# leavesnight/VIEO_SLAM

Hardware: AMD Instinct MI355X
Metric: frontend+localBA frames/sec on EuRoC MH05 stereo-VIO; ATE vs ref (higher is better)
Workload: dtype u8 (extract/match) + f64 (pose optimisation)

## Files before the change

### vieo_slam_amd/csrc/pose_opt_vio.hip

```cpp
#pragma clang fp contract(fast)

#include <type_traits>
#include <vector>

#include "imu_device.h"

namespace vieo {

constexpr double kCosH[9] = {1.0, -0.125, 0.0026041666666666665, -2.170138888888889e-05, 9.68812003968254e-08, -2.691144455467372e-10, 5.096864498991235e-13, -7.001187498614334e-16, 7.292903644389931e-19};
constexpr double kSinHT[9] = {0.5, -0.020833333333333332, 0.00026041666666666666, -1.5500992063492063e-06, 5.382288910934745e-09, -1.2232474797578965e-11, 1.9603324996120133e-14, -2.333729166204778e-17, 2.1449716601146855e-20};
constexpr double kJrA[9] = {0.5, -0.041666666666666664, 0.001388888888888889, -2.48015873015873e-05, 2.755731922398589e-07, -2.08767569878681e-09, 1.1470745597729725e-11, -4.779477332387385e-14, 1.5619206968586225e-16};
constexpr double kJrB[9] = {0.16666666666666666, -0.008333333333333333, 0.0001984126984126984, -2.7557319223985893e-06, 2.505210838544172e-08, -1.6059043836821613e-10, 7.647163731819816e-13, -2.8114572543455206e-15, 8.22063524662433e-18};
constexpr double kAtanQ[16] = {0.3333333333333333, -0.2, 0.14285714285714285, -0.1111111111111111, 0.09090909090909091, -0.07692307692307693, 0.06666666666666667, -0.058823529411764705, 0.05263157894736842, -0.047619047619047616, 0.043478260869565216, -0.04, 0.037037037037037035, -0.034482758620689655, 0.03225806451612903, -0.030303030303030304};
__device__ __forceinline__ Qd q_renorm(const Qd& q, bool& ok) {
  const double e = (q.w * q.w + q.x * q.x + q.y * q.y + q.z * q.z) - 1.0;
  ok = ok && fabs(e) < 1e-5;
  const double r = 1.0 - e * (0.5 - 0.375 * e);
  return Qd{q.w * r, q.x * r, q.y * r, q.z * r};
}
template <int N>
__device__ __forceinline__ double horner(const double (&c)[N], double u) {
  double r = c[N - 1];
#pragma unroll
  for (int k = N - 2; k >= 0; k--) r = __builtin_fma(r, u, c[k]);
  return r;
}
__device__ __forceinline__ double rcp_nr(double d) {
  double inv = __builtin_amdgcn_rcp(d);
  inv = __builtin_fma(__builtin_fma(-d, inv, 1.0), inv, inv);
  return __builtin_fma(__builtin_fma(-d, inv, 1.0), inv, inv);
}
__device__ __forceinline__ Qd so3_exp_unit(const double* w, bool& ok) {
  const double u = w[0] * w[0] + w[1] * w[1] + w[2] * w[2];
  ok = ok && u < 0.25;
  const double real = horner(kCosH, u), imag = horner(kSinHT, u);
  return q_renorm(Qd{real, imag * w[0], imag * w[1], imag * w[2]}, ok);
}
__device__ __forceinline__ void so3_log_unit(const Qd& q, double* out, double* g, bool& ok) {
  const double n2 = q.x * q.x + q.y * q.y + q.z * q.z, w2 = q.w * q.w;
  ok = ok && n2 < 0.0625 * w2;
  const double iw = rcp_nr(q.w), x2 = n2 * (iw * iw);
  const double Q = horner(kAtanQ, x2), P = __builtin_fma(-x2, Q, 1.0);
  const double f = 2.0 * P * iw;
  out[0] = f * q.x, out[1] = f * q.y, out[2] = f * q.z;
  *g = Q * rcp_nr(4.0 * P * P);
}
__device__ __noinline__ double so3_JrInv_g_of(const double* e) {
  const double th2 = e[0] * e[0] + e[1] * e[1] + e[2] * e[2], th = sqrt(th2);
  if (th < 1e-5) return 1. / 12.;
  double sth, cth;
  sincos(th, &sth, &cth);
  return (1.0 - (1.0 + cth) * th / (2.0 * sth)) / th2;
}
__device__ __forceinline__ void so3_JrInv_g(const double* e, double g, double* J) {
  const double xx = e[0] * e[0], yy = e[1] * e[1], zz = e[2] * e[2];
  const double xy = g * e[0] * e[1], xz = g * e[0] * e[2], yz = g * e[1] * e[2];
  J[0] = 1.0 - g * (yy + zz), J[1] = xy - 0.5 * e[2], J[2] = xz + 0.5 * e[1];
  J[3] = xy + 0.5 * e[2], J[4] = 1.0 - g * (xx + zz), J[5] = yz - 0.5 * e[0];
  J[6] = xz - 0.5 * e[1], J[7] = yz + 0.5 * e[0], J[8] = 1.0 - g * (xx + yy);
}
__device__ __forceinline__ void so3_Jr_unit(const double* w, double* J) {
  const double u = w[0] * w[0] + w[1] * w[1] + w[2] * w[2];
  const double A = horner(kJrA, u), B = horner(kJrB, u);
  const double xx = w[0] * w[0], yy = w[1] * w[1], zz = w[2] * w[2];
  const double xy = B * w[0] * w[1], xz = B * w[0] * w[2], yz = B * w[1] * w[2];
  J[0] = 1.0 - B * (yy + zz), J[1] = xy + A * w[2], J[2] = xz - A * w[1];
  J[3] = xy - A * w[2], J[4] = 1.0 - B * (xx + zz), J[5] = yz + A * w[0];
  J[6] = xz + A * w[1], J[7] = yz - A * w[0], J[8] = 1.0 - B * (xx + yy);
}
struct RotCache {
  Qd qe, qb;
  double g_e;
  double w[3];
  Qd qp;
  double g_p;
  int w_small;
};

__device__ __forceinline__ void prior_error(const NSd& pr, const NSd& si, double* err, RotCache& C) {
  double Rb[9], d[3];
  q_to_R(q_of(pr), Rb);
  for (int k = 0; k < 3; k++) d[k] = si.p[k] - pr.p[k];
  mTv3(Rb, d, err);
  bool ok = true;
  Qd q = q_renorm(q_mul(q_conj(q_of(pr)), q_of(si)), ok);
  double g;
  so3_log_unit(q, err + 6, &g, ok);
  for (int k = 0; k < 3; k++) {
    err[3 + k] = si.v[k] - pr.v[k];
    err[9 + k] = si.bg[k] + si.dbg[k] - (pr.bg[k] + pr.dbg[k]);
    err[12 + k] = si.ba[k] + si.dba[k] - (pr.ba[k] + pr.dba[k]);
  }
  if (!ok) {
    q = q_norm(q_mul(q_conj(q_of(pr)), q_of(si)));
    so3_log_q(q, err + 6);
    g = so3_JrInv_g_of(err + 6);
  }
  C.qp = q, C.g_p = g;
}
__device__ __forceinline__ void prior_jacobian_init(double* J, int tid, int nthreads) {
  for (int e = tid; e < 225; e += nthreads) {
    const int r = e / 15, c = e - r * 15;
    J[e] = (r == c && ((r >= 3 && r < 6) || r >= 9)) ? 1.0 : 0.0;
  }
}
__device__ __forceinline__ void prior_linearize(const double* err, double* J, const RotCache& C) {
  double tmp[9], Jrinv[9];
  q_to_R(C.qp, tmp);
  set3(J, 15, 0, 0, tmp, 1.0);
  so3_JrInv_g(err + 6, C.g_p, Jrinv);
  set3(J, 15, 6, 6, Jrinv, 1.0);
}

__device__ __forceinline__ void imu_error_rot(const vieo_imu_preint& M, const Qd& qRij, const NSd& si, const NSd& sj, double* err, RotCache& C) {
  double w[3];
  mv3(M.JgR, si.dbg, w);
  bool ok = true;
  const Qd qx = so3_exp_unit(w, ok);
  const bool w_small = ok;
  Qd qb = q_renorm(q_mul(q_conj(q_of(si)), q_of(sj)), ok);
  const Qd qa = q_renorm(q_mul(qRij, qx), ok);
  Qd qe = q_renorm(q_mul(q_conj(qa), qb), ok);
  double g;
  so3_log_unit(qe, err + 6, &g, ok);
  if (!ok) {
    qb = q_norm(q_mul(q_conj(q_of(si)), q_of(sj)));
    qe = q_norm(q_mul(q_conj(q_norm(q_mul(qRij, so3_exp_q(w)))), qb));
    so3_log_q(qe, err + 6);
    g = so3_JrInv_g_of(err + 6);
  }
  C.qe = qe, C.qb = qb, C.g_e = g;
  C.w[0] = w[0], C.w[1] = w[1], C.w[2] = w[2], C.w_small = w_small ? 1 : 0;
}
__device__ __forceinline__ void imu_jacobian_init(const vieo_imu_preint& M, double* J, int tid, int nthreads) {
  for (int e = tid; e < 9 * 24; e += nthreads) {
    const int r = e / 24, c = e - r * 24;
    double v = 0.0;
    if (r < 3) {
      if (c >= 9 && c < 12) v = (c - 9 == r) ? -1.0 : 0.0;
      if (c >= 18 && c < 21) v = -M.Jgp[r * 3 + c - 18];
      if (c >= 21) v = -M.Jap[r * 3 + c - 21];
    } else if (r < 6) {
      if (c >= 18 && c < 21) v = -M.Jgv[(r - 3) * 3 + c - 18];
      if (c >= 21) v = -M.Jav[(r - 3) * 3 + c - 21];
    }
    J[e] = v;
  }
}
__device__ __forceinline__ void imu_linearize_pv(const vieo_imu_preint& M, const double* gw, const NSd& si, const NSd& sj, double* J) {
  const int ld = 24, cj = 0, ci = 9, idR = 6, idV = 3;
  double Ri[9], RiT[9], Rj[9], t[3], r[3], Hm[9], tmp[9];
  q_to_R(q_of(si), Ri);
// ... 242 lines not shown
struct VioShared {
  NSd nsj, nsi, bkj, bki, prior;
  union {
    struct {
      double H[900], L[900];
    };
    struct {
      double cov[225], C[225], E[225], Cinv[225 * 2];
    };
  };
  double b[32], x[32], tr_tail[64];
  double red[4 * 28], vis[28];
  double errI[9], errB[6], errP[15], wI[9], wP[15];
  double JI[9 * 24], JP[225], InfoI[81], T[225], TP[225], Hp[225];
  double chiq[8];
  double xv[4];
  int xfail;
  RotCache rc;
  double qRij[4];
  double gw[4];
  vieo_imu_preint imu;
  int ok;
};

struct VioEncShared {
  double Info[36], err[6], we[6], chi, J[6 * 12], T[6 * 12];
};

__device__ __noinline__ void vio_enc_setup(const vieo_pose_enc* pe, VioEncShared* S) {
  double M[6][12];
  for (int i = 0; i < 6; i++)
    for (int j = 0; j < 6; j++) M[i][j] = pe->enc.Sigma[i * 6 + j], M[i][6 + j] = (i == j) ? 1.0 : 0.0;
  for (int c = 0; c < 6; c++) {
    int piv = c;
    for (int r = c + 1; r < 6; r++)
      if (fabs(M[r][c]) > fabs(M[piv][c])) piv = r;
    if (piv != c)
      for (int j = 0; j < 12; j++) {
        const double t = M[c][j];
        M[c][j] = M[piv][j], M[piv][j] = t;
      }
    const double d = M[c][c];
    for (int j = 0; j < 12; j++) M[c][j] /= d;
    for (int r = 0; r < 6; r++)
      if (r != c) {
        const double f = M[r][c];
// ... 46 lines not shown
  asm volatile(
      "global_load_dwordx4 %0, %16, off sc0 sc1\n\t"
      "global_load_dwordx4 %1, %16, off offset:512 sc0 sc1\n\t"
      "global_load_dwordx4 %2, %16, off offset:1024 sc0 sc1\n\t"
      "global_load_dwordx4 %3, %16, off offset:1536 sc0 sc1\n\t"
      "global_load_dwordx4 %4, %16, off offset:2048 sc0 sc1\n\t"
      "global_load_dwordx4 %5, %16, off offset:2560 sc0 sc1\n\t"
      "global_load_dwordx4 %6, %16, off offset:3072 sc0 sc1\n\t"
      "global_load_dwordx4 %7, %16, off offset:3584 sc0 sc1\n\t"
      "global_load_dwordx4 %8, %17, off sc0 sc1\n\t"
      "global_load_dwordx4 %9, %17, off offset:512 sc0 sc1\n\t"
      "global_load_dwordx4 %10, %17, off offset:1024 sc0 sc1\n\t"
      "global_load_dwordx4 %11, %17, off offset:1536 sc0 sc1\n\t"
      "global_load_dwordx4 %12, %17, off offset:2048 sc0 sc1\n\t"
      "global_load_dwordx4 %13, %17, off offset:2560 sc0 sc1\n\t"
      "global_load_dwordx4 %14, %17, off offset:3072 sc0 sc1\n\t"
      "global_load_dwordx4 %15, %17, off offset:3584 sc0 sc1\n\t"
      "s_waitcnt vmcnt(0)"
      : "=&v"(v[0]), "=&v"(v[1]), "=&v"(v[2]), "=&v"(v[3]), "=&v"(v[4]), "=&v"(v[5]), "=&v"(v[6]), "=&v"(v[7]), "=&v"(v[8]), "=&v"(v[9]), "=&v"(v[10]), "=&v"(v[11]), "=&v"(v[12]), "=&v"(v[13]), "=&v"(v[14]), "=&v"(v[15])
      : "v"(p), "v"(p2)
      : "memory");
}
template <int BS, bool MC, bool ENC>
__global__ void __launch_bounds__(BS)
k_pose_opt_vio(const vieo_vio_frame* __restrict__ frames, const vieo_pose_obs* __restrict__ obs_all,
               uint8_t* __restrict__ outlier_all, vieo_vio_result* __restrict__ results, int other_launched,
               PoseXchg* __restrict__ xchg, unsigned launch_id) {
  __shared__ VioShared S;
  __shared__ double s_tr[BS == 64 ? 1 : 28 * (BS / 32) * 34];
  __shared__ double s_xf[MC ? 48 * (BS / 64) : 1];
  __shared__ __align__(8) unsigned char s_cam_store[sizeof(CamD) * (MC ? 4 : 1)];
  CamD* s_cams = reinterpret_cast<CamD*>(s_cam_store);
  __shared__ __align__(8) unsigned char s_enc_store[ENC ? sizeof(VioEncShared) : 8];
  VioEncShared* SE = reinterpret_cast<VioEncShared*>(s_enc_store);
  __shared__ __align__(16) vieo_pose_obs s_obs[(BS == 256 && !MC) ? 768 : 1];
  __shared__ uint8_t s_lvl[(BS == 256 && !MC) ? 768 : 4];
  const int f = blockIdx.x, tid = threadIdx.x, lane = tid & 63, wave = tid >> 6;
  const int T1 = BS > 64 ? 64 : 0, T2 = BS > 128 ? 128 : 0;
  const int T3 = BS > 192 ? 192 : 0;
  const vieo_vio_frame& F = frames[f];
  const int N = F.base.n_obs;
  constexpr int kVioSplitObs = 768;
  constexpr int kVioReplicaMinObs = 700;
  const vieo_pose_obs* obs = obs_all + F.base.obs_begin;
  uint8_t* outl = outlier_all + F.base.obs_begin;
  vieo_vio_result* R = results + f;
  const vieo_pose_enc* pe = F.base.enc;
  const bool cam_other = (F.base.n_cams > 0) != MC, enc_other = (pe != nullptr && pe->enc.dt != 0) != ENC;
  if ((cam_other && (other_launched & 1)) || (enc_other && (other_launched & 2))) return;
  const bool other_kind = cam_other || enc_other;
  bool bad_cams = other_kind;
  if (MC && !other_kind) {
    if (tid == 0) S.ok = !(F.base.n_cams > 4 || !F.base.cams);
    __syncthreads();
    if (tid < 4 && S.ok)
      if (!cam_from_abi(F.base.cams[tid < F.base.n_cams ? tid : 0], s_cams[tid])) S.ok = 0;
    __syncthreads();
    bad_cams = !S.ok;
    __syncthreads();
  }
  if (bad_cams || (N < 3 && !F.no_mps) || N > kVioMaxObs) {
    for (int i = tid; i < N; i += BS) outl[i] = 0;
    for (int i = tid; i < 225; i += BS) R->H_marg[i] = 0;
    if (tid == 0) {
      R->base.nav = F.base.nav;
      R->base.n_inliers = 0;
      R->base.status = bad_cams ? VIEO_E_INVALID : N > kVioMaxObs ? VIEO_E_CAPACITY : VIEO_POSE_TOO_FEW;
      R->base.lm_iterations = 0;
      R->base.reserved = 0;
      R->has_marg = 0;
      R->reserved = 0;
    }
    return;
  }
  CamD c;
  c.fx = F.base.fx, c.fy = F.base.fy, c.cx = F.base.cx, c.cy = F.base.cy, c.bf = F.base.bf;
  for (int i = 0; i < 9; i++) c.Rcb[i] = F.base.Rcb[i];
  for (int i = 0; i < 3; i++) c.tcb[i] = F.base.tcb[i];
  const bool fixedLast = !F.last_has_prior, hasImu = F.imu.dt != 0;
  const int n = fixedLast ? 15 : 30;
  const bool bodom = hasImu || ENC;
  if (tid == 0) {
    ns_load(S.nsj, F.base.nav);
    ns_load(S.nsi, F.nav_last);
    ns_load(S.prior, F.nav_prior);
  }
  if (ENC && tid == T2) vio_enc_setup(pe, SE);
  if (hasImu && wave == 0) {
    double* M = S.Cinv;
    for (int e = lane; e < 9 * 18; e += 64) {
      const int i = e / 18, j = e % 18;
      M[e] = j < 9 ? F.imu.Sigma[i * 9 + j] : (j - 9 == i ? 1.0 : 0.0);
    }
    wave_sync();
    for (int cidx = 0; cidx < 9; cidx++) {
      int piv = cidx;
      double best = fabs(M[cidx * 18 + cidx]);
      for (int r = cidx + 1; r < 9; r++)
        if (fabs(M[r * 18 + cidx]) > best) best = fabs(M[r * 18 + cidx]), piv = r;
      if (piv != cidx) {
        if (lane < 18) {
// ... 4 lines not shown
        wave_sync();
      }
      const double d = M[cidx * 18 + cidx];
      wave_sync();
      if (lane < 18) M[cidx * 18 + lane] /= d;
      wave_sync();
      double fr[3];
      for (int h = 0; h < 3; h++) {
        const int e = lane + 64 * h;
        fr[h] = e < 162 ? M[(e / 18) * 18 + cidx] : 0;
      }
      wave_sync();
      for (int h = 0; h < 3; h++) {
        const int e = lane + 64 * h;
        if (e < 162 && e / 18 != cidx) M[e] -= fr[h] * M[cidx * 18 + e % 18];
      }
      wave_sync();
    }
    for (int e = lane; e < 81; e += 64) S.InfoI[e] = M[(e / 9) * 18 + 9 + e % 9] * (fixedLast ? 1e-2 : 1.0);
  }
  if (!fixedLast)
    for (int e = tid; e < 225; e += BS) S.Hp[e] = F.H_prior[e];
  if (tid < 3) S.gw[tid] = F.gw[tid];
  prior_jacobian_init(S.JP, tid, BS);
  if (hasImu) imu_jacobian_init(F.imu, S.JI, tid, BS);
  if (tid == BS - 1 && hasImu) {
    const Qd q = R_to_q(F.imu.Rij);
    S.qRij[0] = q.w, S.qRij[1] = q.x, S.qRij[2] = q.y, S.qRij[3] = q.z;
  }
  for (int e = tid; e < (int)(offsetof(vieo_imu_preint, Sigma) / 8); e += BS)
    reinterpret_cast<double*>(&S.imu)[e] = reinterpret_cast<const double*>(&F.imu)[e];
  __syncthreads();
  if (BS == 256) {
    for (int i = tid; i < 900; i += BS) S.H[i] = 0.0;
    __syncthreads();
  }
  const double deltatij = F.imu.dt ? F.imu.dt : F.dt_frames;
  const double infoBg = F.inv_sigma_bg2 / deltatij * (fixedLast ? 1e-2 : 1.0);
  const double infoBa = F.inv_sigma_ba2 / deltatij * (fixedLast ? 1e-2 : 1.0);
  const double dI = sqrt(16.919), dB = sqrt(12.592), dP = sqrt(25.0), dE = sqrt(12.592);
  const double deltaMono = (double)(float)sqrt(5.991), deltaStereo = (double)(float)sqrt(7.815);
  const float chi2Mono = 5.991f, chi2Stereo = 7.815f;
  auto optimise = [&](auto vt_c, auto g_c) __attribute__((always_inline)) {
  constexpr int VT = decltype(vt_c)::value;
  constexpr int G = decltype(g_c)::value;
  const int g = G > 1 ? (int)blockIdx.y : 0;
  const int Nv = tid < VT ? N : 0;
  const int i0 = g * VT + tid;
// ... 71 lines not shown
        v[tid] = t;
      }
    }
    epoch++;
    __syncthreads();
    if (S.xfail && tid < 64) {
      const unsigned long long pz = (unsigned long long)(((launch_id & 0xFFFFFu) << 12) | 0xFFFu) << 32;
      xq_t pq;
      pq.x = pz, pq.y = pz;
      xq_store(&xb->cell[tid >> 5][g][tid & 31], pq);
    }
  };
  unsigned long long levelmask = 0;
  bool vis_robust = true;
  int nBad = 0, total_iters = 0, total_trials = 0;
  const int n_edges_total = N + (hasImu ? 1 : 0) + 1 + (fixedLast ? 0 : 1) + (ENC ? 1 : 0);
  double rhoE = 1.0;

#ifdef VIEO_POSE_PROBE
  unsigned long long pp_last = __builtin_amdgcn_s_memtime();
#endif
  constexpr int VTE = kObsLds ? 128 : VT;
  auto all_errors = [&](double* rhoI, double* rhoB, double* rhoP, bool with_visual, double* vis) -> double {
    if (with_visual && tid < VTE) {
      Est e;
      e.p[0] = S.nsj.p[0], e.p[1] = S.nsj.p[1], e.p[2] = S.nsj.p[2];
      e.qw = S.nsj.qw, e.qx = S.nsj.qx, e.qy = S.nsj.qy, e.qz = S.nsj.qz;
      PoseXf X;
      make_xf(c, e, X);
      rig_xf(X, e.p);
      double tc = 0;
      if constexpr (kObsLds) {
        const int K = (N + VTE - 1) / VTE;
        auto slots = [&](int k0, auto u_c) __attribute__((always_inline)) {
          constexpr int U = decltype(u_c)::value;
          VisFlat E[U];
          bool valid[U];
#pragma unroll
          for (int u = 0; u < U; u++) {
            const int i = min(tid + (k0 + u) * VTE, N - 1);
            valid[u] = tid + (k0 + u) * VTE < N && !s_lvl[i];
            vis_error_flat(c, X, s_obs[i], valid[u], E[u]);
          }
#pragma unroll
          for (int u = 0; u < U; u++) {
            double r0, r1;
// ... 14 lines not shown
        double err[3], Pc[3];
        const double chi2 = edge_eval<MC>(c, s_cams, X, e.p, o, err, Pc, nullptr, MC ? s_xf + (VT == BS ? 0 : 48 * wave) : nullptr);
        double r0 = chi2, r1 = 1.;
        if (vis_robust) {
          const double dl = o.ur >= 0 ? deltaStereo : deltaMono;
          huber(chi2, dl, dl * dl, &r0, &r1);
        }
        tc += r0;
      }
      }
      tc = BS == 64 ? wave_sum_d_bfly(tc) : wave_sum_d(tc);
      if (lane == 0) S.red[wave] = tc;
    }
    if (BS > 192) {
      if (VT > 128) {
        if (tid == T3 && hasImu) {
          RT(17, imu_error(S.imu, S.gw, S.nsi, S.nsj, S.errI, 6, 1);
             imu_error_rot(S.imu, Qd{S.qRij[0], S.qRij[1], S.qRij[2], S.qRij[3]}, S.nsi, S.nsj, S.errI, S.rc));
        }
      } else {
        if (tid == T3 && hasImu) RT(17, imu_error_rot(S.imu, Qd{S.qRij[0], S.qRij[1], S.qRij[2], S.qRij[3]}, S.nsi, S.nsj, S.errI, S.rc));
        if (tid == T2 && hasImu) RT(18, imu_error(S.imu, S.gw, S.nsi, S.nsj, S.errI, 6, 1));
      }
    } else if (tid == 0 && hasImu) {
      imu_error(S.imu, S.gw, S.nsi, S.nsj, S.errI, 6, 1);
      imu_error_rot(S.imu, Qd{S.qRij[0], S.qRij[1], S.qRij[2], S.qRij[3]}, S.nsi, S.nsj, S.errI, S.rc);
    }
    if (tid == TPr && !fixedLast) RT(19, prior_error(S.prior, S.nsi, S.errP, S.rc));
    if (tid == T2) {
      for (int k = 0; k < 3; k++) {
        S.errB[k] = (S.nsj.bg[k] + S.nsj.dbg[k]) - (S.nsi.bg[k] + S.nsi.dbg[k]);
        S.errB[3 + k] = (S.nsj.ba[k] + S.nsj.dba[k]) - (S.nsi.ba[k] + S.nsi.dba[k]);
      }
      if (ENC) vio_enc_eval(pe, SE, &S.nsi, &S.nsj, 0);
    }
    constexpr bool kTail = BS == 256 && VT == 192 && !ENC;
    if (kTail) {
      if (wave == 3 && hasImu) {
        wave_sync();
        if (lane < 9) {
          double t = 0;
#pragma unroll
          for (int j = 0; j < 9; j++) t += S.InfoI[lane * 9 + j] * S.errI[j];
          S.wI[lane] = t;
        }
        wave_sync();
        if (lane == 0) {
          double eI = 0;
#pragma unroll
          for (int i = 0; i < 9; i++) eI += S.errI[i] * S.wI[i];
          double r0 = eI, r1 = 1.0;
          if (fixedLast) huber(eI, dI, dI * dI, &r0, &r1);
          S.chiq[0] = r0, S.chiq[1] = r1;
        }
      }
      if (wave == 2) {
// ... 91 lines not shown
      double r0;
      huber(SE->chi, dE, dE * dE, &r0, &rhoE);
      chi += r0;
    }
    if (with_visual) {
      double v = S.red[0];
      for (int w = 1; w < VTE / 64; w++) v += S.red[w];
      *vis = G > 1 ? S.xv[0] : v;
    }
    return chi;
  };

  for (int it = 0; it < 4; it++) {
    __syncthreads();
    if (!bodom && tid == 0) {
      ns_load(S.nsj, F.base.nav);
      if (!fixedLast) ns_load(S.nsi, F.nav_last);
    }
    __syncthreads();
    double lambda = -1, ni = 2;
    int nBadLM = 0;
    double accChi = 0, accI = 1, accB = 1, accP = 1, accE = 1;
    for (int iter = 0; iter < 10; iter++) {
      total_iters++;
      double rhoI, rhoB, rhoP;
      PP(0);
      double chiG;
      if (iter == 0)
        chiG = all_errors(&rhoI, &rhoB, &rhoP, false, nullptr);
      else
        chiG = accChi, rhoI = accI, rhoB = accB, rhoP = accP, rhoE = accE;
      PP(1);
      double acc[28];
#pragma unroll
      for (int i = 0; i < 28; i++) acc[i] = 0;
      if (tid < VT) {
      Est e;
      e.p[0] = S.nsj.p[0], e.p[1] = S.nsj.p[1], e.p[2] = S.nsj.p[2];
      e.qw = S.nsj.qw, e.qx = S.nsj.qx, e.qy = S.nsj.qy, e.qz = S.nsj.qz;
      PoseXf X;
      make_xf(c, e, X);
      rig_xf(X, e.p);
      if constexpr (kObsLds) {
        const int K = (N + VT - 1) / VT;
        auto slots = [&](int k0, auto u_c) __attribute__((always_inline)) {
          constexpr int U = decltype(u_c)::value;
          VisFlat E[U];
          bool valid[U];
          double J[U][18];
#pragma unroll
          for (int u = 0; u < U; u++) {
            const int i = tid + (k0 + u) * VT;
            valid[u] = i < N && !((levelmask >> (k0 + u)) & 1);
            const vieo_pose_obs o = s_obs[min(i, N - 1)];
            vis_error_flat(c, X, o, valid[u], E[u]);
            vis_jacobian_flat(c, X, e.p, o, E[u], J[u]);
          }
#pragma unroll
          for (int u = 0; u < U; u++) {
            double r0, r1;
            const double dl = E[u].stereo ? deltaStereo : deltaMono;
            huber_flat(E[u].chi2, dl, dl * dl, vis_robust, &r0, &r1);
            acc[27] += valid[u] ? r0 : 0.0;
            vis_accumulate_flat(J[u], E[u].err, valid[u] ? E[u].info : 0.0, r1, acc);
          }
        };
        int k = 0;
        for (; k + 1 < K; k += 2) slots(k, std::integral_constant<int, 2>{});
        if (k < K) slots(k, std::integral_constant<int, 1>{});
      } else {
      vieo_pose_obs o_next = ld_obs(min(i0, N - 1));
      for (int k = 0, i = i0; i < Nv; k++, i += GV) {
        const vieo_pose_obs o = o_next;
        if (i + GV < N) o_next = ld_obs(i + GV);
        if ((levelmask >> k) & 1) continue;
        double err[3], Pc[3];
        double J[18];
        const double chi2 = edge_eval<MC>(c, s_cams, X, e.p, o, err, Pc, J, MC ? s_xf + (VT == BS ? 0 : 48 * wave) : nullptr);
        const bool stereo = o.ur >= 0;
        double r0 = chi2, r1 = 1.;
        if (vis_robust) {
          const double dl = stereo ? deltaStereo : deltaMono;
          huber(chi2, dl, dl * dl, &r0, &r1);
        }
        acc[27] += r0;
        visual_accumulate(J, err, (double)o.inv_sigma2, r1, stereo, acc);
      }
      }
      }
      constexpr bool kOverlap = BS == 256;
      if (BS > 192) {
        if (wave == 3) {
          if (hasImu) {
            if (lane == 0) {
              RT(20, imu_linearize_pv(S.imu, S.gw, S.nsi, S.nsj, S.JI);
// ... 37 lines not shown
              H10 = __builtin_amdgcn_mfma_f64_16x16x4f64(bJ[1][ks], T0[ks], H10, 0, 0, 0);
              H11 = __builtin_amdgcn_mfma_f64_16x16x4f64(bJ[1][ks], T1[ks], H11, 0, 0, 0);
            }
            const int m = fixedLast ? 9 : 24;
#pragma unroll
            for (int r = 0; r < 4; r++) {
              const int row = l4 + 4 * r;
              {
                const int c1 = row, c2 = l15;
                if (c1 < m && c2 <= c1) S.H[(c1 < 9 ? c1 : c1 + 6) * n + (c2 < 9 ? c2 : c2 + 6)] = 0.0 + H00[r];
                if (c1 < m && l15 == 8) S.b[c1 < 9 ? c1 : c1 + 6] = 0.0 + H01[r];
              }
              if (!fixedLast) {
                const int c1 = 16 + row;
                if (c1 < 24) {
                  S.H[(c1 + 6) * n + (l15 < 9 ? l15 : l15 + 6)] = 0.0 + H10[r];
                  if (l15 < 8 && 16 + l15 <= c1) S.H[(c1 + 6) * n + 16 + l15 + 6] = 0.0 + H11[r];
                  if (l15 == 8) S.b[c1 + 6] = 0.0 + H11[r];
                }
              }
            }
          }
        }
      } else if (hasImu) {
        for (int i = lane; i < 9 * 24; i += 64) S.JI[i] = 0;
        wave_sync();
        if (tid == 0) {
          imu_linearize(S.imu, S.gw, S.nsi, S.nsj, S.errI, S.JI, 6, 3, 1);
          imu_linearize_rot(S.imu, S.errI, S.JI, S.rc);
        }
      }
      if (tid == TPr && !fixedLast) RT(22, prior_linearize(S.errP, S.JP, S.rc));
      if (kOverlap && wave == (TPr >> 6) && !fixedLast) {
        wave_sync();
        typedef double v4d __attribute__((ext_vector_type(4)));
        const int l15 = lane & 15, l4 = lane >> 4;
        double aP[4], bP[4];
#pragma unroll
        for (int ks = 0; ks < 4; ks++) {
          const int k = 4 * ks + l4;
          aP[ks] = (l15 < 15 && k < 15) ? rhoP * S.Hp[l15 * 15 + k] : 0.0;
          bP[ks] = (l15 < 15 && k < 15) ? S.JP[k * 15 + l15] : 0.0;
        }
        v4d TPv = {0, 0, 0, 0}, HPv = {0, 0, 0, 0};
#pragma unroll
        for (int ks = 0; ks < 4; ks++) TPv = __builtin_amdgcn_mfma_f64_16x16x4f64(aP[ks], bP[ks], TPv, 0, 0, 0);
        if (l15 == 15) {
#pragma unroll
          for (int r = 0; r < 4; r++) {
            const int k = 4 * r + l4;
            TPv[r] = k < 15 ? -S.wP[k] * rhoP : 0.0;
          }
        }
#pragma unroll
        for (int ks = 0; ks < 4; ks++) HPv = __builtin_amdgcn_mfma_f64_16x16x4f64(bP[ks], TPv[ks], HPv, 0, 0, 0);
#pragma unroll
        for (int r = 0; r < 4; r++) {
          const int row = l4 + 4 * r;
          if (row < 15) S.L[l15 < 15 ? row * 15 + l15 : 225 + row] = HPv[r];
        }
      }
      if (ENC && tid == T2) vio_enc_eval(pe, SE, &S.nsi, &S.nsj, 1);
      PP(2);
      block_sum_lds<28, BS>(acc, BS == 64 ? S.H : s_tr, S.vis, tid);
      grid_sum(S.vis, 28);
      PP(3);
      double currentChi = chiG + S.vis[27];
      const double iniChi = currentChi;
      const double rhoE0 = rhoE;
      PP(4);
      if (!kOverlap && hasImu) {
        const int cnt = fixedLast ? 81 : 216;
        for (int eidx = tid; eidx < cnt; eidx += BS) {
          const int a = fixedLast ? eidx / 9 : eidx / 24, cc = eidx - a * (fixedLast ? 9 : 24);
          double t = 0;
#pragma unroll
          for (int q = 0; q < 9; q++) t += (rhoI * S.InfoI[a * 9 + q]) * S.JI[q * 24 + cc];
          S.T[a * 24 + cc] = t;
        }
      }
      if (!kOverlap && !fixedLast)
        for (int eidx = tid; eidx < 225; eidx += BS) {
          const int a = eidx / 15, cc = eidx % 15;
          double t = 0;
#pragma unroll
          for (int q = 0; q < 15; q++) t += (rhoP * S.Hp[a * 15 + q]) * S.JP[q * 15 + cc];
          S.TP[a * 15 + cc] = t;
        }
// ... 87 lines not shown
          double t = 0;
          for (int a = 0; a < 6; a++) t += SE->J[a * 12 + c1] * SE->T[a * 12 + c2];
          const int s1 = (c1 < 6 ? 0 : 9) + c1 + (c1 % 6 < 3 ? 0 : 3), s2 = (c2 < 6 ? 0 : 9) + c2 + (c2 % 6 < 3 ? 0 : 3);
          if (!kOverlap || s1 >= s2) S.H[s1 * n + s2] += t;
        }
        if (tid < nc) {
          double t = 0;
          for (int a = 0; a < 6; a++) t += SE->J[a * 12 + tid] * (-SE->we[a] * rhoE0);
          S.b[(tid < 6 ? 0 : 9) + tid + (tid % 6 < 3 ? 0 : 3)] += t;
        }
        __syncthreads();
      }
      PP(5);
      if (iter == 0) {
        double mx = 0;
        for (int j = 0; j < n; j++) mx = fmax(fabs(S.H[j * n + j]), mx);
        lambda = 1e-5 * mx;
        ni = 2;
        nBadLM = 0;
      }
      double rho = 0;
      int qmax = 0;
      do {
        __syncthreads();
        if (tid >= BS - 64) {
          constexpr int kNs = (int)(sizeof(NSd) / 8);
          if (lane < kNs) ((double*)&S.bkj)[lane] = ((const double*)&S.nsj)[lane];
          if (lane < kNs && BS == 64) ((double*)&S.bki)[lane] = ((const double*)&S.nsi)[lane];
          if (BS > 64 && lane >= 32 && lane < 32 + kNs) ((double*)&S.bki)[lane - 32] = ((const double*)&S.nsi)[lane - 32];
        }
        if (BS == 64) wave_sync();
        PP(11);
        if (wave == 0) {
          const bool ok = n == 15 ? wave_solve_vio<9>((const lds_f64*)S.H, n, lambda, (const lds_f64*)S.b, (lds_f64*)S.x, (lds_f64*)S.L, lane)
                                  : wave_solve_vio<24>((const lds_f64*)S.H, n, lambda, (const lds_f64*)S.b, (lds_f64*)S.x, (lds_f64*)S.L, lane);
          if (lane == 0) S.ok = ok ? 1 : 0;
        }
        PP(12);
        __syncthreads();
        PP(6);
        const bool ok2 = S.ok != 0;
        if (!ok2) {
          if (tid < n) S.x[tid] = 0;
          __syncthreads();
        }
        if (tid == 0) ns_inc_unit(S.nsj, S.x, S.x + 9);
        if (tid == T1 && !fixedLast) ns_inc_unit(S.nsi, S.x + 15, S.x + 24);
        if (tid == T2) {
          double sc = 0;
          if (fixedLast) {
#pragma unroll
            for (int j = 0; j < 15; j++) sc += S.x[j] * (lambda * S.x[j] + S.b[j]);
          } else {
#pragma unroll
            for (int j = 0; j < 30; j++) sc += S.x[j] * (lambda * S.x[j] + S.b[j]);
          }
          S.chiq[6] = sc;
        }
        __syncthreads();
        PP(7);
        double r1, r2, r3, visChi;
        const double tempChiG = all_errors(&r1, &r2, &r3, true, &visChi);
        double tempChi = tempChiG + visChi;
        PP(9);
        if (!ok2) tempChi = DBL_MAX;
        rho = currentChi - tempChi;
        double scale = S.chiq[6];
        scale += 1e-3;
        rho /= scale;
        if (rho > 0 && isfinite(tempChi)) {
          const double r21 = 2 * rho - 1;
          double alpha = 1. - r21 * r21 * r21;
          alpha = fmin(alpha, 2. / 3.);
          lambda *= fmax(1. / 3., alpha);
          ni = 2;
          currentChi = tempChi;
          accChi = tempChiG, accI = r1, accB = r2, accP = r3, accE = rhoE;
        } else {
          lambda *= ni;
          ni *= 2;
          __syncthreads();
          {
            constexpr int kNs = (int)(sizeof(NSd) / 8);
            if (tid < kNs) ((double*)&S.nsj)[tid] = ((const double*)&S.bkj)[tid];
            if (tid >= 32 && tid < 32 + kNs) ((double*)&S.nsi)[tid - 32] = ((const double*)&S.bki)[tid - 32];
          }
        }
        qmax++;
        total_trials++;
      } while (rho < 0 && qmax < 10);
      __syncthreads();
      if (qmax == 10 || rho == 0) break;
      if ((iniChi - currentChi) * 1e3 < iniChi)
        nBadLM++;
      else
        nBadLM = 0;
      if (nBadLM >= 3) break;
    }
    PP(10);
    __syncthreads();
    Est e;
    e.p[0] = S.nsj.p[0], e.p[1] = S.nsj.p[1], e.p[2] = S.nsj.p[2];
    e.qw = S.nsj.qw, e.qx = S.nsj.qx, e.qy = S.nsj.qy, e.qz = S.nsj.qz;
    PoseXf X;
    make_xf(c, e, X);
    rig_xf(X, e.p);
    const float chi2close = (float)(1.5 * (double)chi2Mono);
    double nb[1] = {0};
    for (int k = 0, i = i0; i < Nv; k++, i += GV) {
      const vieo_pose_obs o = ld_obs(i);
      double err[3], Pc[3];
      const float chi2 = (float)edge_eval<MC>(c, s_cams, X, e.p, o, err, Pc, nullptr, MC ? s_xf + (VT == BS ? 0 : 48 * wave) : nullptr);
      bool bad;
      if (o.ur < 0)
        bad = chi2 > ((o.flags & 1) ? chi2close : chi2Mono) || !(Pc[2] > 0.);
      else
        bad = chi2 > chi2Stereo;
      if (bad) {
        levelmask |= (1ull << k);
        nb[0] += 1;
      } else
        levelmask &= ~(1ull << k);
// ... 23 lines not shown
    for (int k = 0, i = i0; i < Nv; k++, i += GV) {
      const vieo_pose_obs o = ld_obs(i);
      double err[3], Pc[3];
      const double chi2 = edge_eval<MC>(c, s_cams, X, e.p, o, err, Pc, nullptr, MC ? s_xf + (VT == BS ? 0 : 48 * wave) : nullptr);
      if (chi2 < (double)(o.ur < 0 ? 18.f : 24.f)) {
        levelmask &= ~(1ull << k);
        outmask &= ~(1ull << k);
        if constexpr (kObsLds) s_lvl[i] = 0;
      } else
        nb[0] += 1;
    }
    block_sum_bs<1, BS>(nb, S.red, tid);
    if (G > 1) {
      __syncthreads();
      if (tid == 0) S.xv[0] = nb[0];
      __syncthreads();
      grid_sum(S.xv, 1);
      nb[0] = S.xv[0];
    }
    nBad = (int)nb[0];
  }
  for (int k = 0, i = i0; i < Nv; k++, i += GV) outl[i] = (outmask >> k) & 1;
  if (F.compute_marg) {
    double rhoI, rhoB, rhoP;
    all_errors(&rhoI, &rhoB, &rhoP, false, nullptr);
    Est e;
    e.p[0] = S.nsj.p[0], e.p[1] = S.nsj.p[1], e.p[2] = S.nsj.p[2];
    e.qw = S.nsj.qw, e.qx = S.nsj.qx, e.qy = S.nsj.qy, e.qz = S.nsj.qz;
    PoseXf X;
    make_xf(c, e, X);
    rig_xf(X, e.p);
    double acc[27];
#pragma unroll
    for (int i = 0; i < 27; i++) acc[i] = 0;
    vieo_pose_obs o_next = ld_obs(min(i0, N - 1));
    for (int k = 0, i = i0; i < Nv; k++, i += GV) {
      const vieo_pose_obs o = o_next;
      if (i + GV < N) o_next = ld_obs(i + GV);
      if ((levelmask >> k) & 1) continue;
      double err[3], Pc[3];
      double J[18];
      const double chi2 = edge_eval<MC>(c, s_cams, X, e.p, o, err, Pc, J, MC ? s_xf + (VT == BS ? 0 : 48 * wave) : nullptr);
      const bool stereo = o.ur >= 0;
      double r0 = chi2, r1 = 1.;
      if (vis_robust) {
        const double dl = stereo ? deltaStereo : deltaMono;
        huber(chi2, dl, dl * dl, &r0, &r1);
      }
      visual_accumulate(J, err, (double)o.inv_sigma2, r1, stereo, acc);
    }
    block_sum_bs<27, BS>(acc, S.red, tid);
    for (int i = tid; i < 9 * 24; i += BS) S.JI[i] = 0;
    __syncthreads();
    if (tid < 27) {
      double v = 0;
#pragma unroll
      for (int t = 0; t < 27; t++)
        if (tid == t) v = acc[t];
      S.vis[tid] = v;
    }
    if (BS > 192) {
      if (tid == 0 && hasImu) imu_linearize(S.imu, S.gw, S.nsi, S.nsj, S.errI, S.JI, 6, 3, 1);
      if (tid == T3 && hasImu) imu_linearize_rot(S.imu, S.errI, S.JI, S.rc);
    } else if (tid == 0 && hasImu) {
      imu_linearize(S.imu, S.gw, S.nsi, S.nsj, S.errI, S.JI, 6, 3, 1);
      imu_linearize_rot(S.imu, S.errI, S.JI, S.rc);
    }
    if (tid == T1 && !fixedLast) prior_linearize(S.errP, S.JP, S.rc);
    if (ENC && tid == T2) vio_enc_eval(pe, SE, &S.nsi, &S.nsj, 1);
    for (int i = tid; i < 225; i += BS) S.cov[i] = 0, S.C[i] = 0, S.E[i] = 0;
    __syncthreads();
    grid_sum(S.vis, 27);
    if (tid < 36) {
      const int a = tid / 6, bq = tid % 6;
      const int lo = a < bq ? a : bq, hi = a < bq ? bq : a;
      const int t = lo * 6 - lo * (lo - 1) / 2 + (hi - lo);
      S.cov[(a < 3 ? a : a + 3) * 15 + (bq < 3 ? bq : bq + 3)] = S.vis[t];
    }
    __syncthreads();
    if (hasImu) {
      for (int eidx = tid; eidx < 9 * 24; eidx += BS) {
        const int a = eidx / 24, cc = eidx % 24;
        double t = 0;
        for (int q = 0; q < 9; q++) t += (rhoI * S.InfoI[a * 9 + q]) * S.JI[q * 24 + cc];
        S.T[a * 24 + cc] = t;
      }
      __syncthreads();
      for (int eidx = tid; eidx < 24 * 24; eidx += BS) {
        const int c1 = eidx / 24, c2 = eidx % 24;
        double t = 0;
        for (int a = 0; a < 9; a++) t += S.JI[a * 24 + c1] * S.T[a * 24 + c2];
// ... 220 lines not shown
  if (narrow && !MC)
    hipLaunchKernelGGL((k_pose_opt_vio<64, MC, ENC>), dim3(n_frames), dim3(64), 0, stream, d_frames, d_obs,
                       d_outlier, d_results, others, (PoseXchg*)nullptr, 0u);
  else {
    unsigned launch_id = 0;
    PoseXchg* xb = replicas ? vio_xchg_records(stream, kVioReplicaFrames, &launch_id) : nullptr;
    if (xb) {
      const char* drop = getenv("VIEO_POSE_REPLICA_DROP");
      if (drop && atoi(drop) > 0) launch_id |= 0x80000000u;
    }
    hipLaunchKernelGGL((k_pose_opt_vio<256, MC, ENC>), dim3(n_frames, xb ? kXG : 1), dim3(256), 0, stream, d_frames, d_obs,
                       d_outlier, d_results, others, xb, launch_id);
  }
}

extern "C" {

int vieo_pose_set_replicas(int on) {
  const int was = vio_replicas();
  vio_replicas() = on ? 1 : 0;
  return was;
}

static int vio_launch(const vieo_vio_frame* d_frames, int n_frames, const vieo_pose_obs* d_obs,
                      uint8_t* d_outlier, vieo_vio_result* d_results, int which, int which_enc, void* stream) {
  if (!d_frames || n_frames <= 0 || !d_obs || !d_outlier || !d_results) return VIEO_E_INVALID;
  int rc = require_device();
  if (rc != VIEO_OK) return rc;
  static const int forced = [] {
    const char* e = getenv("VIEO_POSE_THREADS");
    return e ? atoi(e) : 0;
  }();
  const bool narrow = forced == 64 || (forced != 256 && n_frames > 256);
  const int others = (which == 3 ? 1 : 0) | (which_enc == 3 ? 2 : 0);
  hipStream_t st = (hipStream_t)stream;
  if ((which & 1) && (which_enc & 1)) vio_launch_kind<false, false>(narrow, d_frames, n_frames, d_obs, d_outlier, d_results, others, st);
  if ((which & 2) && (which_enc & 1)) vio_launch_kind<true, false>(narrow, d_frames, n_frames, d_obs, d_outlier, d_results, others, st);
  if ((which & 1) && (which_enc & 2)) vio_launch_kind<false, true>(narrow, d_frames, n_frames, d_obs, d_outlier, d_results, others, st);
  if ((which & 2) && (which_enc & 2)) vio_launch_kind<true, true>(narrow, d_frames, n_frames, d_obs, d_outlier, d_results, others, st);
  VIEO_HIP_CHECK(hipGetLastError());
  return VIEO_OK;
}

int vieo_pose_optimization_vio_batch_device(const vieo_vio_frame* d_frames, int n_frames,
                                            const vieo_pose_obs* d_obs, uint8_t* d_outlier,
                                            vieo_vio_result* d_results, void* stream) {
// ... 71 lines not shown
```

Before: 62800.

## Shrink narrow VIO pose kernel LDS and register footprint for higher residency

For the 64-thread batch variant, adds a compact shared-memory layout that aliases the Jacobian, backup and IMU buffers. It moves the serial error, linearize and retract work into noinline lane functions, parks LM state in LDS across those calls, and keeps the camera record in LDS. It also sets launch bounds to request two blocks per execution unit. The goal is to cut register pressure and LDS usage so more frames are resident per CU, at the cost of extra LDS traffic, syncs and call overhead, plus the correctness risk of aliased buffers.

```diff
diff --git a/vieo_slam_amd/csrc/pose_opt_vio.hip b/vieo_slam_amd/csrc/pose_opt_vio.hip
--- a/vieo_slam_amd/csrc/pose_opt_vio.hip
+++ b/vieo_slam_amd/csrc/pose_opt_vio.hip
@@ -45,13 +45,14 @@
   out[0] = f * q.x, out[1] = f * q.y, out[2] = f * q.z;
   *g = Q * rcp_nr(4.0 * P * P);
 }
-__device__ __noinline__ double so3_JrInv_g_of(const double* e) {
+__device__ __forceinline__ double so3_JrInv_g_of_inl(const double* e) {
   const double th2 = e[0] * e[0] + e[1] * e[1] + e[2] * e[2], th = sqrt(th2);
   if (th < 1e-5) return 1. / 12.;
   double sth, cth;
   sincos(th, &sth, &cth);
   return (1.0 - (1.0 + cth) * th / (2.0 * sth)) / th2;
 }
+__device__ __noinline__ double so3_JrInv_g_of(const double* e) { return so3_JrInv_g_of_inl(e); }
 __device__ __forceinline__ void so3_JrInv_g(const double* e, double g, double* J) {
   const double xx = e[0] * e[0], yy = e[1] * e[1], zz = e[2] * e[2];
   const double xy = g * e[0] * e[1], xz = g * e[0] * e[2], yz = g * e[1] * e[2];
@@ -77,6 +78,7 @@
   int w_small;
 };
 
+template <bool LEAF = false>
 __device__ __forceinline__ void prior_error(const NSd& pr, const NSd& si, double* err, RotCache& C) {
   double Rb[9], d[3];
   q_to_R(q_of(pr), Rb);
@@ -94,7 +96,7 @@
   if (!ok) {
     q = q_norm(q_mul(q_conj(q_of(pr)), q_of(si)));
     so3_log_q(q, err + 6);
-    g = so3_JrInv_g_of(err + 6);
+    g = LEAF ? so3_JrInv_g_of_inl(err + 6) : so3_JrInv_g_of(err + 6);
   }
   C.qp = q, C.g_p = g;
 }
@@ -112,6 +114,7 @@
   set3(J, 15, 6, 6, Jrinv, 1.0);
 }
 
+template <bool LEAF = false>
 __device__ __forceinline__ void imu_error_rot(const vieo_imu_preint& M, const Qd& qRij, const NSd& si, const NSd& sj, double* err, RotCache& C) {
   double w[3];
   mv3(M.JgR, si.dbg, w);
@@ -127,7 +130,7 @@
     qb = q_norm(q_mul(q_conj(q_of(si)), q_of(sj)));
     qe = q_norm(q_mul(q_conj(q_norm(q_mul(qRij, so3_exp_q(w)))), qb));
     so3_log_q(qe, err + 6);
-    g = so3_JrInv_g_of(err + 6);
+    g = LEAF ? so3_JrInv_g_of_inl(err + 6) : so3_JrInv_g_of(err + 6);
   }
   C.qe = qe, C.qb = qb, C.g_e = g;
   C.w[0] = w[0], C.w[1] = w[1], C.w[2] = w[2], C.w_small = w_small ? 1 : 0;
@@ -416,6 +419,69 @@
   vieo_imu_preint imu;
   int ok;
 };
+
+struct VioSharedNarrow {
+  NSd nsj, nsi, prior;
+  union {
+    struct {
+      double H[900], L[900];
+    };
+    struct {
+      double cov[225], C[225], E[225], Cinv[225 * 2];
+    };
+    struct {
+      double pad_l_[900], JI[9 * 24], pad_ji_[9], JP[225], T[225], TP[225];
+    };
+    struct {
+      double pad_bk_[900 + 24 * 34];
+      NSd bkj, bki;
+    };
+  };
+  double b[32], x[32], tr_tail[64];
+  double red[4], vis[28];
+  double InfoI[81], Hp[225];
+  union {
+    vieo_imu_preint imu;
+    struct {
+      double pad_imu_[offsetof(vieo_imu_preint, Sigma) / 8];
+      double errI[9], errB[6], errP[15], wI[9], wP[15], chiq[8], xv[4], park[8];
+    };
+  };
+  int xfail;
+  RotCache rc;
+  double qRij[4];
+  double gw[4];
+  int ok;
+};
+static_assert(sizeof(NSd) == 22 * 8 && 2 * sizeof(NSd) <= (900 - 24 * 34) * 8, "the backups fit behind the column buffers");
+static_assert(sizeof(VioSharedNarrow) <= 20480 - 208 - 16, "eight frames per CU (with the camera record beside it)");
+
+typedef __attribute__((address_space(3))) VioSharedNarrow lds_vio;
+__device__ __noinline__ void vio_lane_errors(lds_vio* Sl, int hasImu, int fixedLast) {
+  VioSharedNarrow& S = *(VioSharedNarrow*)Sl;
+  if (hasImu) {
+    imu_error(S.imu, S.gw, S.nsi, S.nsj, S.errI, 6, 1);
+    imu_error_rot<true>(S.imu, Qd{S.qRij[0], S.qRij[1], S.qRij[2], S.qRij[3]}, S.nsi, S.nsj, S.errI, S.rc);
+  }
+  if (!fixedLast) prior_error<true>(S.prior, S.nsi, S.errP, S.rc);
+  for (int k = 0; k < 3; k++) {
+    S.errB[k] = (S.nsj.bg[k] + S.nsj.dbg[k]) - (S.nsi.bg[k] + S.nsi.dbg[k]);
+    S.errB[3 + k] = (S.nsj.ba[k] + S.nsj.dba[k]) - (S.nsi.ba[k] + S.nsi.dba[k]);
+  }
+}
+__device__ __noinline__ void vio_lane_linearize(lds_vio* Sl, int hasImu, int fixedLast) {
+  VioSharedNarrow& S = *(VioSharedNarrow*)Sl;
+  if (hasImu) {
+    imu_linearize(S.imu, S.gw, S.nsi, S.nsj, S.errI, S.JI, 6, 3, 1);
+    imu_linearize_rot(S.imu, S.errI, S.JI, S.rc);
+  }
+  if (!fixedLast) prior_linearize(S.errP, S.JP, S.rc);
+}
+__device__ __noinline__ void vio_lane_retract(lds_vio* Sl, int fixedLast) {
+  VioSharedNarrow& S = *(VioSharedNarrow*)Sl;
+  ns_inc_unit(S.nsj, S.x, S.x + 9);
+  if (!fixedLast) ns_inc_unit(S.nsi, S.x + 15, S.x + 24);
+}
 
 struct VioEncShared {
   double Info[36], err[6], we[6], chi, J[6 * 12], T[6 * 12];
@@ -508,11 +574,11 @@
       : "memory");
 }
 template <int BS, bool MC, bool ENC>
-__global__ void __launch_bounds__(BS)
+__global__ void __launch_bounds__(BS, BS == 64 ? 2 : 1)
 k_pose_opt_vio(const vieo_vio_frame* __restrict__ frames, const vieo_pose_obs* __restrict__ obs_all,
                uint8_t* __restrict__ outlier_all, vieo_vio_result* __restrict__ results, int other_launched,
                PoseXchg* __restrict__ xchg, unsigned launch_id) {
-  __shared__ VioShared S;
+  __shared__ std::conditional_t<BS == 64, VioSharedNarrow, VioShared> S;
   __shared__ double s_tr[BS == 64 ? 1 : 28 * (BS / 32) * 34];
   __shared__ double s_xf[MC ? 48 * (BS / 64) : 1];
   __shared__ __align__(8) unsigned char s_cam_store[sizeof(CamD) * (MC ? 4 : 1)];
@@ -522,6 +588,14 @@
   __shared__ __align__(16) vieo_pose_obs s_obs[(BS == 256 && !MC) ? 768 : 1];
   __shared__ uint8_t s_lvl[(BS == 256 && !MC) ? 768 : 4];
   const int f = blockIdx.x, tid = threadIdx.x, lane = tid & 63, wave = tid >> 6;
+  auto phase_tid = [&]() -> int {
+    int t = tid;
+    if (BS == 64) {
+      asm volatile("" : "+v"(t));
+      __builtin_assume(t >= 0 && t < 64);
+    }
+    return t;
+  };
   const int T1 = BS > 64 ? 64 : 0, T2 = BS > 128 ? 128 : 0;
   const int T3 = BS > 192 ? 192 : 0;
   const vieo_vio_frame& F = frames[f];
@@ -559,10 +633,13 @@
     }
     return;
   }
-  CamD c;
-  c.fx = F.base.fx, c.fy = F.base.fy, c.cx = F.base.cx, c.cy = F.base.cy, c.bf = F.base.bf;
-  for (int i = 0; i < 9; i++) c.Rcb[i] = F.base.Rcb[i];
-  for (int i = 0; i < 3; i++) c.tcb[i] = F.base.tcb[i];
+  CamD c_regs;
+  c_regs.fx = F.base.fx, c_regs.fy = F.base.fy, c_regs.cx = F.base.cx, c_regs.cy = F.base.cy, c_regs.bf = F.base.bf;
+  for (int i = 0; i < 9; i++) c_regs.Rcb[i] = F.base.Rcb[i];
+  for (int i = 0; i < 3; i++) c_regs.tcb[i] = F.base.tcb[i];
+  constexpr bool kCamLds = BS == 64 && !MC;
+  if (kCamLds && tid == 0) s_cams[0] = c_regs;
+  const CamD& c = kCamLds ? s_cams[0] : c_regs;
   const bool fixedLast = !F.last_has_prior, hasImu = F.imu.dt != 0;
   const int n = fixedLast ? 15 : 30;
   const bool bodom = hasImu || ENC;
@@ -613,8 +690,10 @@
   if (!fixedLast)
     for (int e = tid; e < 225; e += BS) S.Hp[e] = F.H_prior[e];
   if (tid < 3) S.gw[tid] = F.gw[tid];
-  prior_jacobian_init(S.JP, tid, BS);
-  if (hasImu) imu_jacobian_init(F.imu, S.JI, tid, BS);
+  if (BS > 64) {
+    prior_jacobian_init(S.JP, tid, BS);
+    if (hasImu) imu_jacobian_init(F.imu, S.JI, tid, BS);
+  }
   if (tid == BS - 1 && hasImu) {
     const Qd q = R_to_q(F.imu.Rij);
     S.qRij[0] = q.w, S.qRij[1] = q.x, S.qRij[2] = q.y, S.qRij[3] = q.z;
@@ -732,6 +811,8 @@
 #endif
   constexpr int VTE = kObsLds ? 128 : VT;
   auto all_errors = [&](double* rhoI, double* rhoB, double* rhoP, bool with_visual, double* vis) -> double {
+    const int tid = phase_tid(), lane = tid & 63;
+    const int Nv = tid < VT ? N : 0, i0 = g * VT + tid;
     if (with_visual && tid < VTE) {
       Est e;
       e.p[0] = S.nsj.p[0], e.p[1] = S.nsj.p[1], e.p[2] = S.nsj.p[2];
@@ -792,16 +873,19 @@
         if (tid == T3 && hasImu) RT(17, imu_error_rot(S.imu, Qd{S.qRij[0], S.qRij[1], S.qRij[2], S.qRij[3]}, S.nsi, S.nsj, S.errI, S.rc));
         if (tid == T2 && hasImu) RT(18, imu_error(S.imu, S.gw, S.nsi, S.nsj, S.errI, 6, 1));
       }
+    } else if constexpr (BS == 64) {
+      if (tid == 0) vio_lane_errors((lds_vio*)&S, hasImu, fixedLast);
     } else if (tid == 0 && hasImu) {
       imu_error(S.imu, S.gw, S.nsi, S.nsj, S.errI, 6, 1);
       imu_error_rot(S.imu, Qd{S.qRij[0], S.qRij[1], S.qRij[2], S.qRij[3]}, S.nsi, S.nsj, S.errI, S.rc);
     }
-    if (tid == TPr && !fixedLast) RT(19, prior_error(S.prior, S.nsi, S.errP, S.rc));
+    if (BS > 64 && tid == TPr && !fixedLast) RT(19, prior_error(S.prior, S.nsi, S.errP, S.rc));
     if (tid == T2) {
-      for (int k = 0; k < 3; k++) {
-        S.errB[k] = (S.nsj.bg[k] + S.nsj.dbg[k]) - (S.nsi.bg[k] + S.nsi.dbg[k]);
-        S.errB[3 + k] = (S.nsj.ba[k] + S.nsj.dba[k]) - (S.nsi.ba[k] + S.nsi.dba[k]);
-      }
+      if (BS > 64)
+        for (int k = 0; k < 3; k++) {
+          S.errB[k] = (S.nsj.bg[k] + S.nsj.dbg[k]) - (S.nsi.bg[k] + S.nsi.dbg[k]);
+          S.errB[3 + k] = (S.nsj.ba[k] + S.nsj.dba[k]) - (S.nsi.ba[k] + S.nsi.dba[k]);
+        }
       if (ENC) vio_enc_eval(pe, SE, &S.nsi, &S.nsj, 0);
     }
     constexpr bool kTail = BS == 256 && VT == 192 && !ENC;
@@ -939,15 +1023,25 @@
     int nBadLM = 0;
     double accChi = 0, accI = 1, accB = 1, accP = 1, accE = 1;
     for (int iter = 0; iter < 10; iter++) {
+      const int tid = phase_tid(), lane = tid & 63;
+      const int Nv = tid < VT ? N : 0, i0 = g * VT + tid;
       total_iters++;
       double rhoI, rhoB, rhoP;
       PP(0);
       double chiG;
       if (iter == 0)
         chiG = all_errors(&rhoI, &rhoB, &rhoP, false, nullptr);
+      else if (BS > 64)
+        chiG = accChi, rhoI = accI, rhoB = accB, rhoP = accP, rhoE = accE;
       else
-        chiG = accChi, rhoI = accI, rhoB = accB, rhoP = accP, rhoE = accE;
+        chiG = rhoI = rhoB = rhoP = 0;
       PP(1);
+      if constexpr (BS == 64) {
+        if (tid == 0) {
+          S.park[0] = lambda, S.park[1] = ni;
+          if (iter == 0) S.park[2] = chiG, S.park[3] = rhoI, S.park[4] = rhoB, S.park[5] = rhoP, S.park[6] = rhoE;
+        }
+      }
       double acc[28];
 #pragma unroll
       for (int i = 0; i < 28; i++) acc[i] = 0;
@@ -988,6 +1082,7 @@
       } else {
       vieo_pose_obs o_next = ld_obs(min(i0, N - 1));
       for (int k = 0, i = i0; i < Nv; k++, i += GV) {
+        if (kCamLds) asm volatile("" ::: "memory");
         const vieo_pose_obs o = o_next;
         if (i + GV < N) o_next = ld_obs(i + GV);
         if ((levelmask >> k) & 1) continue;
@@ -1071,7 +1166,7 @@
             }
           }
         }
-      } else if (hasImu) {
+      } else if (BS > 64 && hasImu) {
         for (int i = lane; i < 9 * 24; i += 64) S.JI[i] = 0;
         wave_sync();
         if (tid == 0) {
@@ -1079,7 +1174,7 @@
           imu_linearize_rot(S.imu, S.errI, S.JI, S.rc);
         }
       }
-      if (tid == TPr && !fixedLast) RT(22, prior_linearize(S.errP, S.JP, S.rc));
+      if (BS > 64 && tid == TPr && !fixedLast) RT(22, prior_linearize(S.errP, S.JP, S.rc));
       if (kOverlap && wave == (TPr >> 6) && !fixedLast) {
         wave_sync();
         typedef double v4d __attribute__((ext_vector_type(4)));
@@ -1113,6 +1208,16 @@
       PP(2);
       block_sum_lds<28, BS>(acc, BS == 64 ? S.H : s_tr, S.vis, tid);
       grid_sum(S.vis, 28);
+      if constexpr (BS == 64) {
+        if (!fixedLast) prior_jacobian_init(S.JP, tid, BS);
+        if (hasImu)
+          for (int i = lane; i < 9 * 24; i += 64) S.JI[i] = 0;
+        wave_sync();
+        if (tid == 0) vio_lane_linearize((lds_vio*)&S, hasImu, fixedLast);
+        __syncthreads();
+        lambda = S.park[0], ni = S.park[1], chiG = S.park[2], rhoI = S.park[3], rhoB = S.park[4], rhoP = S.park[5];
+        rhoE = S.park[6];
+      }
       PP(3);
       double currentChi = chiG + S.vis[27];
       const double iniChi = currentChi;
@@ -1246,6 +1351,7 @@
       double rho = 0;
       int qmax = 0;
       do {
+        const int tid = phase_tid(), lane = tid & 63;
         __syncthreads();
         if (tid >= BS - 64) {
           constexpr int kNs = (int)(sizeof(NSd) / 8);
@@ -1268,8 +1374,12 @@
           if (tid < n) S.x[tid] = 0;
           __syncthreads();
         }
-        if (tid == 0) ns_inc_unit(S.nsj, S.x, S.x + 9);
-        if (tid == T1 && !fixedLast) ns_inc_unit(S.nsi, S.x + 15, S.x + 24);
+        if constexpr (BS == 64) {
+          if (tid == 0) vio_lane_retract((lds_vio*)&S, fixedLast);
+        } else {
+          if (tid == 0) ns_inc_unit(S.nsj, S.x, S.x + 9);
+          if (tid == T1 && !fixedLast) ns_inc_unit(S.nsi, S.x + 15, S.x + 24);
+        }
         if (tid == T2) {
           double sc = 0;
           if (fixedLast) {
@@ -1299,7 +1409,10 @@
           lambda *= fmax(1. / 3., alpha);
           ni = 2;
           currentChi = tempChi;
-          accChi = tempChiG, accI = r1, accB = r2, accP = r3, accE = rhoE;
+          if constexpr (BS > 64)
+            accChi = tempChiG, accI = r1, accB = r2, accP = r3, accE = rhoE;
+          else if (tid == 0)
+            S.park[2] = tempChiG, S.park[3] = r1, S.park[4] = r2, S.park[5] = r3, S.park[6] = rhoE;
         } else {
           lambda *= ni;
           ni *= 2;
@@ -1322,6 +1435,8 @@
       if (nBadLM >= 3) break;
     }
     PP(10);
+    const int tid = phase_tid();
+    const int Nv = tid < VT ? N : 0, i0 = g * VT + tid;
     __syncthreads();
     Est e;
     e.p[0] = S.nsj.p[0], e.p[1] = S.nsj.p[1], e.p[2] = S.nsj.p[2];
@@ -1391,6 +1506,8 @@
   }
   for (int k = 0, i = i0; i < Nv; k++, i += GV) outl[i] = (outmask >> k) & 1;
   if (F.compute_marg) {
+    const int tid = phase_tid(), lane = tid & 63;
+    const int Nv = tid < VT ? N : 0, i0 = g * VT + tid;
     double rhoI, rhoB, rhoP;
     all_errors(&rhoI, &rhoB, &rhoP, false, nullptr);
     Est e;
@@ -1420,6 +1537,7 @@
     }
     block_sum_bs<27, BS>(acc, S.red, tid);
     for (int i = tid; i < 9 * 24; i += BS) S.JI[i] = 0;
+    if (BS == 64 && !fixedLast) prior_jacobian_init(S.JP, tid, BS);
     __syncthreads();
     if (tid < 27) {
       double v = 0;
@@ -1431,11 +1549,13 @@
     if (BS > 192) {
       if (tid == 0 && hasImu) imu_linearize(S.imu, S.gw, S.nsi, S.nsj, S.errI, S.JI, 6, 3, 1);
       if (tid == T3 && hasImu) imu_linearize_rot(S.imu, S.errI, S.JI, S.rc);
+    } else if constexpr (BS == 64) {
+      if (tid == 0) vio_lane_linearize((lds_vio*)&S, hasImu, fixedLast);
     } else if (tid == 0 && hasImu) {
       imu_linearize(S.imu, S.gw, S.nsi, S.nsj, S.errI, S.JI, 6, 3, 1);
       imu_linearize_rot(S.imu, S.errI, S.JI, S.rc);
     }
-    if (tid == T1 && !fixedLast) prior_linearize(S.errP, S.JP, S.rc);
+    if (BS > 64 && tid == T1 && !fixedLast) prior_linearize(S.errP, S.JP, S.rc);
     if (ENC && tid == T2) vio_enc_eval(pe, SE, &S.nsi, &S.nsj, 1);
     for (int i = tid; i < 225; i += BS) S.cov[i] = 0, S.C[i] = 0, S.E[i] = 0;
     __syncthreads();
@@ -1702,6 +1822,13 @@
   return was;
 }
 
+int vieo_debug_pose_vio_batch_residency(void) {
+  if (require_device() != VIEO_OK) return -1;
+  int per_cu = 0;
+  if (hipOccupancyMaxActiveBlocksPerMultiprocessor(&per_cu, k_pose_opt_vio<64, false, false>, 64, 0) != hipSuccess) return -1;
+  return per_cu;
+}
+
 static int vio_launch(const vieo_vio_frame* d_frames, int n_frames, const vieo_pose_obs* d_obs,
                       uint8_t* d_outlier, vieo_vio_result* d_results, int which, int which_enc, void* stream) {
   if (!d_frames || n_frames <= 0 || !d_obs || !d_outlier || !d_results) return VIEO_E_INVALID;
```

Result: faster. 64420 (median of 6 runs) (+2.6%).
